# kkrt-labs/stwo-brainfuck

Hardware: AMD Instinct MI355X
Metric: trace cells committed+proved/sec (higher is better)
Workload: dtype u32 (M31 / QM31 modular arithmetic)

## Files before the change

### bindings/rust/bfhip_sys.rs

```rust
#![allow(non_camel_case_types, dead_code)]
use std::ffi::{c_char, c_void};

#[repr(C)] pub struct BfhipCtx { _private: [u8; 0] }
#[repr(C)] pub struct BfhipTrace { _private: [u8; 0] }
#[repr(C)] #[derive(Clone, Copy, Default, Debug, PartialEq, Eq)] pub struct BfhipConventions { pub merkle_node_hash: u32, pub mix_u64: u32, pub logup_mask_order: u32, pub merkle_channel: u32, pub reserved: [u32; 4] }
#[repr(C)] #[derive(Clone, Copy, Debug, PartialEq, Eq)] pub struct BfhipPcsConfig { pub pow_bits: u32, pub log_blowup_factor: u32, pub log_last_layer_degree_bound: u32, pub n_queries: u32, pub reserved: [u32; 4] }
#[repr(C)] pub struct BfhipLocalGroup { _private: [u8; 0] }
#[repr(C)] pub struct BfhipPool { _private: [u8; 0] }

#[link(name = "bfhip")]
extern "C" {
    pub fn bfhip_last_error() -> *const c_char;
    pub fn bfhip_device_count() -> i32;
    pub fn bfhip_device_memory(device_id: i32, free_bytes: *mut u64, total_bytes: *mut u64) -> i32;
    pub fn bfhip_ctx_create(device_id: i32, max_log_domain: u32, out: *mut *mut BfhipCtx) -> i32;
    pub fn bfhip_ctx_destroy(ctx: *mut BfhipCtx) -> i32;
    pub fn bfhip_ctx_sync(ctx: *mut BfhipCtx) -> i32;
    pub fn bfhip_ctx_set_overlap(ctx: *mut BfhipCtx, mask: u32) -> i32;
    pub fn bfhip_ctx_memory(ctx: *mut BfhipCtx, out: *mut u64) -> i32;
    pub fn bfhip_ctx_set_sync_policy(ctx: *mut BfhipCtx, blocking: i32) -> i32;
    pub fn bfhip_ctx_set_mailbox(ctx: *mut BfhipCtx, mode: i32, timeout_ms: u32, test_delay_ms: i32) -> i32;
    pub fn bfhip_ctx_set_conventions(ctx: *mut BfhipCtx, conv: *const BfhipConventions) -> i32;
    pub fn bfhip_ctx_get_conventions(ctx: *mut BfhipCtx, out: *mut BfhipConventions) -> i32;
    pub fn bfhip_ctx_set_pcs_config(ctx: *mut BfhipCtx, pcs: *const BfhipPcsConfig) -> i32;
// ... 2 lines not shown
    pub fn bfhip_free(ctx: *mut BfhipCtx, ptr_d: *mut c_void) -> i32;
    pub fn bfhip_upload(ctx: *mut BfhipCtx, dst_d: *mut c_void, src_h: *const c_void, bytes: usize) -> i32;
    pub fn bfhip_download(ctx: *mut BfhipCtx, dst_h: *mut c_void, src_d: *const c_void, bytes: usize) -> i32;
    pub fn bfhip_memset_zero(ctx: *mut BfhipCtx, dst_d: *mut c_void, bytes: usize) -> i32;
    pub fn bfhip_twiddles(ctx: *mut BfhipCtx, tw_d: *mut *const u32, itw_d: *mut *const u32, root_log: *mut u32) -> i32;
    pub fn bfhip_interpolate(ctx: *mut BfhipCtx, src_cols_h: *const *mut u32, dst_cols_h: *const *mut u32, n_cols: u32, log_size: u32, replicated: i32) -> i32;
    pub fn bfhip_evaluate(ctx: *mut BfhipCtx, coeff_cols_h: *const *mut u32, dst_cols_h: *const *mut u32, n_cols: u32, log_size: u32, log_eval: u32, replicated: i32) -> i32;
    pub fn bfhip_is_first_coeffs(ctx: *mut BfhipCtx, log_min: u32, log_max: u32, dst_cols_h: *const *mut u32) -> i32;
    pub fn bfhip_broadcast16(ctx: *mut BfhipCtx, rows_d: *const u32, dst_d: *mut u32, n_rows: usize) -> i32;
    pub fn bfhip_bit_reverse(ctx: *mut BfhipCtx, src_d: *const u32, dst_d: *mut u32, log_size: u32) -> i32;
    pub fn bfhip_batch_inverse_m31(ctx: *mut BfhipCtx, src_d: *const u32, dst_d: *mut u32, n: usize) -> i32;
    pub fn bfhip_batch_inverse_qm31(ctx: *mut BfhipCtx, src_d: *const *const u32, dst_d: *const *mut u32, n: usize) -> i32;
    pub fn bfhip_accumulate(ctx: *mut BfhipCtx, dst_d: *mut u32, src_d: *const u32, n: usize) -> i32;
    pub fn bfhip_eval_at_point(ctx: *mut BfhipCtx, coeffs_d: *const u32, log_size: u32, replicated: i32, point_h: *const u32, out_h: *mut u32) -> i32;
    pub fn bfhip_merkle_commit_layer(ctx: *mut BfhipCtx, log_size: u32, prev_layer_d: *const c_void, cols_h: *const *const u32, col_shifts_h: *const u32, n_cols: u32, out_hashes_d: *mut c_void) -> i32;
    pub fn bfhip_merkle_commit_layer_poseidon252(ctx: *mut BfhipCtx, log_size: u32, prev_layer_d: *const c_void, cols_h: *const *const u32, col_shifts_h: *const u32, n_cols: u32, out_hashes_d: *mut c_void) -> i32;
    pub fn bfhip_hades_permutation(ctx: *mut BfhipCtx, in_h: *const u32, out_h: *mut u32) -> i32;
    pub fn bfhip_fold_line(ctx: *mut BfhipCtx, src_d: *const *const u32, dst_d: *const *mut u32, log_size: u32, alpha_h: *const u32) -> i32;
    pub fn bfhip_fold_circle_into_line(ctx: *mut BfhipCtx, dst_d: *const *mut u32, src_d: *const *const u32, log_size: u32, alpha_h: *const u32) -> i32;
    pub fn bfhip_grind(ctx: *mut BfhipCtx, digest_h: *const u8, pow_bits: u32, nonce: *mut u64) -> i32;
    pub fn bfhip_gather(ctx: *mut BfhipCtx, col_d: *const u32, idx_h: *const u64, n: usize, out_h: *mut u32) -> i32;
    pub fn bfhip_component_shape(component: i32, n_main_cols: *mut u32, n_logup_cols: *mut u32, n_constraints: *mut u32) -> i32;
    pub fn bfhip_logup_generate(ctx: *mut BfhipCtx, component: i32, log_size: u32, main_rows_h: *const *const u32, lookup_h: *const u32, out_cols_h: *const *mut u32, claimed_sum_h: *mut u32) -> i32;
    pub fn bfhip_eval_constraints(ctx: *mut BfhipCtx, component: i32, log_size: u32, is_first_d: *const u32, main_lde_h: *const *const u32, main_shifts_h: *const u32, inter_lde_h: *const *const u32, inter_shifts_h: *const u32, lookup_h: *const u32, claimed_sum_h: *const u32, coeffs_h: *const u32, acc_d: *const *mut u32) -> i32;
    pub fn bfhip_accumulate_quotients(ctx: *mut BfhipCtx, log_size: u32, cols_h: *const *const u32, col_shifts_h: *const u32, n_cols: u32, n_samples_h: *const u32, sample_points_h: *const u32, sample_values_h: *const u32, random_coeff_h: *const u32, out_d: *const *mut u32) -> i32;
    pub fn bfhip_prove_brainfuck(ctx: *mut BfhipCtx, code: *const c_char, input_h: *const u8, n_input: usize, log_max_rows: u32, proof_json: *mut *mut c_char, proof_len: *mut usize, transcript: *mut *mut c_char, phase_seconds: *mut f64) -> i32;
    pub fn bfhip_free_host(p: *mut c_void);
    pub fn bfhip_ctx_last_proof_flags(ctx: *mut BfhipCtx, flags: *mut u32) -> i32;
    pub fn bfhip_local_group_create(count: u32, out: *mut *mut BfhipLocalGroup) -> i32;
    pub fn bfhip_local_group_destroy(group: *mut BfhipLocalGroup) -> i32;
// ... 42 lines not shown
```

### include/bfhip.h

```cpp
#ifndef BFHIP_H
#define BFHIP_H
#include <stdint.h>
#include <stddef.h>

#ifdef __cplusplus
extern "C" {
#endif

typedef struct bfhip_ctx bfhip_ctx;
typedef struct bfhip_trace bfhip_trace;

enum { BFHIP_MERKLE_STWO_COMPRESS = 0, BFHIP_MERKLE_RFC7693 = 1 };
enum { BFHIP_MIX_U64_COMPRESS = 0, BFHIP_MIX_U64_HASH = 1 };
enum { BFHIP_LOGUP_MASK_CUR_PREV = 0, BFHIP_LOGUP_MASK_PREV_CUR = 1 };
enum { BFHIP_CHANNEL_BLAKE2S = 0, BFHIP_CHANNEL_POSEIDON252 = 1 };
typedef struct bfhip_conventions {
    uint32_t merkle_node_hash;
    uint32_t mix_u64;
    uint32_t logup_mask_order;
    uint32_t merkle_channel;
    uint32_t reserved[4];
} bfhip_conventions;

const char* bfhip_last_error(void);
// ... 32 lines not shown

int32_t bfhip_interpolate(bfhip_ctx* ctx, uint32_t* const* src_cols_h, uint32_t* const* dst_cols_h, uint32_t n_cols, uint32_t log_size, int32_t replicated);
int32_t bfhip_evaluate(bfhip_ctx* ctx, uint32_t* const* coeff_cols_h, uint32_t* const* dst_cols_h, uint32_t n_cols, uint32_t log_size, uint32_t log_eval, int32_t replicated);

int32_t bfhip_is_first_coeffs(bfhip_ctx* ctx, uint32_t log_min, uint32_t log_max, uint32_t* const* dst_cols_h);


int32_t bfhip_broadcast16(bfhip_ctx* ctx, const uint32_t* rows_d, uint32_t* dst_d, size_t n_rows);
int32_t bfhip_bit_reverse(bfhip_ctx* ctx, const uint32_t* src_d, uint32_t* dst_d, uint32_t log_size);
int32_t bfhip_batch_inverse_m31(bfhip_ctx* ctx, const uint32_t* src_d, uint32_t* dst_d, size_t n);
int32_t bfhip_batch_inverse_qm31(bfhip_ctx* ctx, const uint32_t* const src_d[4], uint32_t* const dst_d[4], size_t n);
int32_t bfhip_accumulate(bfhip_ctx* ctx, uint32_t* dst_d, const uint32_t* src_d, size_t n);
int32_t bfhip_eval_at_point(bfhip_ctx* ctx, const uint32_t* coeffs_d, uint32_t log_size, int32_t replicated, const uint32_t point_h[8], uint32_t out_h[4]);
int32_t bfhip_merkle_commit_layer(bfhip_ctx* ctx, uint32_t log_size, const void* prev_layer_d, const uint32_t* const* cols_h, const uint32_t* col_shifts_h,
                                  uint32_t n_cols, void* out_hashes_d);
int32_t bfhip_merkle_commit_layer_poseidon252(bfhip_ctx* ctx, uint32_t log_size, const void* prev_layer_d, const uint32_t* const* cols_h,
                                             const uint32_t* col_shifts_h, uint32_t n_cols, void* out_hashes_d);
int32_t bfhip_hades_permutation(bfhip_ctx* ctx, const uint32_t in_h[24], uint32_t out_h[24]);
int32_t bfhip_fold_line(bfhip_ctx* ctx, const uint32_t* const src_d[4], uint32_t* const dst_d[4], uint32_t log_size, const uint32_t alpha_h[4]);
int32_t bfhip_fold_circle_into_line(bfhip_ctx* ctx, uint32_t* const dst_d[4], const uint32_t* const src_d[4], uint32_t log_size, const uint32_t alpha_h[4]);
int32_t bfhip_grind(bfhip_ctx* ctx, const uint8_t digest_h[32], uint32_t pow_bits, uint64_t* nonce);
int32_t bfhip_gather(bfhip_ctx* ctx, const uint32_t* col_d, const uint64_t* idx_h, size_t n, uint32_t* out_h);


int32_t bfhip_component_shape(int32_t component, uint32_t* n_main_cols, uint32_t* n_logup_cols, uint32_t* n_constraints);
int32_t bfhip_logup_generate(bfhip_ctx* ctx, int32_t component, uint32_t log_size, const uint32_t* const* main_rows_h, const uint32_t lookup_h[24],
                             uint32_t* const* out_cols_h, uint32_t claimed_sum_h[4]);
int32_t bfhip_eval_constraints(bfhip_ctx* ctx, int32_t component, uint32_t log_size, const uint32_t* is_first_d, const uint32_t* const* main_lde_h,
                               const uint32_t* main_shifts_h, const uint32_t* const* inter_lde_h, const uint32_t* inter_shifts_h, const uint32_t lookup_h[24],
                               const uint32_t claimed_sum_h[4], const uint32_t* coeffs_h, uint32_t* const acc_d[4]);
// ... 76 lines not shown
```

### stwo-brainfuck_amd/__init__.py

```python
import ctypes
import os
import weakref

import numpy as np

_HERE = os.path.dirname(os.path.abspath(__file__))
_LIB_PATH = os.environ.get("BFHIP_LIBRARY") or os.path.join(_HERE, "libbfhip.so")
TESTHOOKS_LIBRARY = os.path.join(_HERE, "libbfhip_testhooks.so")
_lib = None

P = (1 << 31) - 1


class BfhipError(RuntimeError):
    pass


def lib():
    global _lib
    if _lib is None:
        if not os.path.exists(_LIB_PATH):
            raise BfhipError(f"{_LIB_PATH} is missing: build it with __graft_entry__.build(); there is no CPU fallback")
        _lib = ctypes.CDLL(_LIB_PATH)
        _lib.bfhip_last_error.restype = ctypes.c_char_p
# ... 250 lines not shown
    def bit_reverse(self, src_ptr, dst_ptr, log_size):
        _check(lib().bfhip_bit_reverse(self._h, ctypes.c_void_p(src_ptr), ctypes.c_void_p(dst_ptr), log_size))

    def batch_inverse_m31(self, src_ptr, dst_ptr, n):
        _check(lib().bfhip_batch_inverse_m31(self._h, ctypes.c_void_p(src_ptr), ctypes.c_void_p(dst_ptr), ctypes.c_size_t(n)))

    def batch_inverse_qm31(self, src_ptrs, dst_ptrs, n):
        _check(lib().bfhip_batch_inverse_qm31(self._h, self._ptr_array(src_ptrs), self._ptr_array(dst_ptrs), ctypes.c_size_t(n)))

    def accumulate(self, dst_ptr, src_ptr, n):
        _check(lib().bfhip_accumulate(self._h, ctypes.c_void_p(dst_ptr), ctypes.c_void_p(src_ptr), ctypes.c_size_t(n)))

    def merkle_commit_layer(self, log_size, prev_ptr, col_ptrs, out_ptr, col_shifts=None):
        sh = None if col_shifts is None else (ctypes.c_uint32 * len(col_shifts))(*col_shifts)
        _check(lib().bfhip_merkle_commit_layer(self._h, log_size, ctypes.c_void_p(prev_ptr) if prev_ptr else None, self._ptr_array(col_ptrs), sh, len(col_ptrs), ctypes.c_void_p(out_ptr)))

    def merkle_commit_layer_poseidon252(self, log_size, prev_ptr, col_ptrs, out_ptr, col_shifts=None):
        sh = None if col_shifts is None else (ctypes.c_uint32 * len(col_shifts))(*col_shifts)
        _check(lib().bfhip_merkle_commit_layer_poseidon252(self._h, log_size, ctypes.c_void_p(prev_ptr) if prev_ptr else None, self._ptr_array(col_ptrs), sh, len(col_ptrs), ctypes.c_void_p(out_ptr)))

    def hades_permutation(self, state3):
        words = []
        for x in state3:
            words += [(int(x) >> (32 * i)) & 0xFFFFFFFF for i in range(8)]
        out = (ctypes.c_uint32 * 24)()
        _check(lib().bfhip_hades_permutation(self._h, (ctypes.c_uint32 * 24)(*words), out))
        return [sum(int(out[8 * k + i]) << (32 * i) for i in range(8)) for k in range(3)]

    def fold_line(self, src_ptrs, dst_ptrs, log_size, alpha4):
        _check(lib().bfhip_fold_line(self._h, self._ptr_array(src_ptrs), self._ptr_array(dst_ptrs), log_size, (ctypes.c_uint32 * 4)(*[int(v) for v in alpha4])))
# ... 217 lines not shown
```

### stwo-brainfuck_amd/csrc/api.hip

```cpp
#include "../../include/bfhip.h"
#include "ctx.h"
#include <cstdlib>
#include "host/circle.h"
#include "host/quotients.h"
#include <cstdio>
#include <vector>
#include <algorithm>
#include <chrono>

using namespace bf;

static thread_local std::string g_err;
void bfhip_set_error(const std::string& s) { g_err = s; }

#define API_TRY try {
#define API_CTX(ctx) try { if (!(ctx)) throw HipError("null context"); (ctx)->c.bind();
#define API_CATCH } catch (const std::exception& e) { g_err = e.what(); return -1; } catch (...) { g_err = "unknown error"; return -1; }

namespace bf {

void Ctx::ensure_aux() { for (auto& a : aux) if (!a) BF_HIP(hipStreamCreateWithFlags(&a, hipStreamNonBlocking)); }
void Ctx::ensure_side() { if (!stream2) BF_HIP(hipStreamCreateWithFlags(&stream2, hipStreamNonBlocking)); }

void Ctx::init(int dev, u32 max_log_domain, const Ctx* tables_from) {
// ... 767 lines not shown
        case 9: r = q_mul_const(x, q_const(y)); break;
        default: r = q_inv(x); break;
    }
    out[4 * i] = r.a.a; out[4 * i + 1] = r.a.b; out[4 * i + 2] = r.b.a; out[4 * i + 3] = r.b.b;
}
extern "C" int32_t bfhip_test_field_op(bfhip_ctx* ctx, uint32_t op, const uint32_t* a_d, const uint32_t* b_d, uint32_t* out_d, size_t n) {
    API_CTX(ctx)
    if (op > 10) throw HipError("bfhip_test_field_op: unknown op");
    if (!a_d || !b_d || !out_d) throw HipError("null argument");
    if (n == 0 || n > (size_t(1) << 28)) throw HipError("bfhip_test_field_op: n out of range");
    hipLaunchKernelGGL(k_test_field_op, dim3((u32)((n + 255) / 256)), dim3(256), 0, ctx->c.stream, op, a_d, b_d, out_d, (u32)n);
    BF_HIP(hipGetLastError());
    return 0;
    API_CATCH
}
extern "C" int32_t bfhip_test_constraint_group_rows(int32_t component, uint32_t log_size, uint32_t main_shift) {
    if (component < 0 || component >= N_COMPONENTS) { g_err = "unknown component"; return -1; }
    ConstraintLaunch L{};
    for (u32 j = 0; j < n_main_cols(component); j++) L.trace[j].shift = main_shift;
    for (u32 j = 0; j + 4 < 4 * n_logup_cols(component); j++) L.inter[j].shift = main_shift;
    L.log_size = log_size;
    return (int32_t)constraint_group_rows(L, component);
}
#endif
```

### stwo-brainfuck_amd/csrc/ctx.h

```cpp
#pragma once
#include <cstdlib>
#include <thread>
#include <chrono>
#include "kernels.h"
#include "comm.h"
#include <memory>
#include <vector>
#include <string>
#include <stdexcept>
#include <cstring>

namespace bf {

struct HipError : std::runtime_error { using std::runtime_error::runtime_error; };
#define BF_HIP(expr) do { hipError_t e__ = (expr); if (e__ != hipSuccess) { (void)hipGetLastError(); throw bf::HipError(std::string(#expr) + ": " + hipGetErrorString(e__)); } } while (0)

struct Arena {
    struct Chunk { char* base; size_t size, used; };
    std::vector<Chunk> chunks;
    size_t chunk_bytes = size_t(1) << 30;
    size_t total_used = 0, peak = 0;
    void* alloc(size_t bytes) {
        bytes = (bytes + 255) & ~size_t(255);
        for (auto& c : chunks) if (c.size - c.used >= bytes) { void* p = c.base + c.used; c.used += bytes; total_used += bytes; if (total_used > peak) peak = total_used; return p; }
// ... 34 lines not shown
    void ensure_aux();
    hipStream_t id_main = nullptr;
    hipStream_t aux_of(hipStream_t s) const { return s == id_main ? aux[0] : aux[1]; }
    hipEvent_t evp[32] = {};
    u32 evp_next = 0;
    hipEvent_t next_event() { return evp[evp_next++ % 32]; }
    u32* d_counters = nullptr;
    u32* merkle_counter() { return d_counters + 64 * (stream == id_main ? 0 : stream == aux[0] ? 1 : stream == aux[1] ? 2 : 3); }
    hipEvent_t ev[6] = {nullptr, nullptr, nullptr, nullptr, nullptr, nullptr};
    u32 tw_root_log = 0;
    u32* d_tw = nullptr; u32* d_itw = nullptr;
    bool owns_tables = true;
    const struct SharedPreprocessed* shared_pre = nullptr;
    uint2* d_tlo = nullptr; uint2* d_thi = nullptr;
    Arena arena;
    char* h_small = nullptr; size_t h_small_bytes = 256 << 10;
    char* d_small_alias = nullptr; char* d_hstage_alias = nullptr;
    template <class T> T* small_alias(T* host_ptr) const { return reinterpret_cast<T*>(d_small_alias + (reinterpret_cast<char*>(host_ptr) - h_small)); }
    char* h_stage = nullptr; char* d_stage = nullptr; size_t stage_bytes = 8 << 20, stage_used = 0;
    u32 last_proof_flags = 0;
    u32 proof_seq = 0;
    int mailbox_mode = -1;
    bool use_mailbox = false;
    int mailboxes_pending = 0;
    double mailbox_timeout = 10.0;
    int mailbox_test_delay_ms = 0;
    u32* flag_host(int k) const { return reinterpret_cast<u32*>(h_small + 3072 + 64 * k); }
    u32* stamp_host(int k) const { return reinterpret_cast<u32*>(h_small + 3584 + 64 * k); }
    u32* mailbox_err_host() const { return reinterpret_cast<u32*>(h_small + 3520); }
    hipEvent_t reap_ev[64] = {}; u32 reap_head = 0, reap_tail = 0;
// ... 147 lines not shown
```

### stwo-brainfuck_amd/csrc/kernels.h

```cpp
#pragma once
#include <hip/hip_runtime.h>
#include "m31.h"
#include "air.h"
#include <string>
#include <vector>

namespace bf {

struct ColDesc { const u32* ptr; u32 shift; u32 pad_; };

int prof_mode(hipStream_t s);
void prof_enable(hipStream_t s, int mode);
void prof_run_begin(hipStream_t s, const char* name);
void prof_run_end(hipStream_t s);
void prof_begin(hipStream_t s, const char* name, double bytes, double units, double aux = 0.0);
void prof_end(hipStream_t s);
void prof_reset(hipStream_t s);
std::string prof_report_json(const hipStream_t* streams, int n);
void prof_forget(hipStream_t s);
struct ProfScope {
    hipStream_t s; bool on;
    ProfScope(hipStream_t s_, const char* name, double bytes, double units = 0.0, bool dominant = false, double aux = 0.0) : s(s_) {
        int m = prof_mode(s);
        on = m == 1 || (m == 2 && dominant);
// ... 43 lines not shown
    const u32* tw;
    u32 block0, grid_x;
    u32 kind;
};
struct FftLaunch { int kind; u32 first_group, ngroups, total_blocks; double bytes, alg, bfly; };
struct FftPlan { bool inverse = false; std::vector<PassArgs> groups; std::vector<FftLaunch> launches; const PassArgs* d_groups = nullptr; };
void fft_plan(FftPlan& plan, bool inverse, const FftJob* jobs, size_t njobs, const u32* tw, const u32* itw, u32 tw_root_log);
void fft_run(hipStream_t stream, const FftPlan& plan);

struct IsFirstCols { u32* ptr[28]; u32 log_min, log_max; };
void is_first_coeffs(hipStream_t stream, const IsFirstCols& a, const u32* itw, u32 tw_root_log);

void merkle_layer(hipStream_t stream, void* out, const void* prev, const ColDesc* d_cols, u32 ncols, u32 log, double col_bytes, u32 out_shift, u32 prev_shift,
                  u32 node_conv, u32 first = 0, u32 count = 0);
struct MerkleTreeDesc { uint4* layers[32]; u32 shifts[32]; u32 col_off[32]; const ColDesc* cols; u32 n_cols, max_log; };
static constexpr u32 MERKLE_SUBTREE_ROOT_LEVEL = 9;
void merkle_subtree(hipStream_t stream, const MerkleTreeDesc& tree, u32 hi, u32 node_conv, double bytes, double compressions);
void merkle_subtree_share(hipStream_t stream, const MerkleTreeDesc& tree, u32 hi, u32 stop, u32 lo, u32 wg0, u32 n_wg, u32 node_conv, double bytes, double compressions);
void merkle_top(hipStream_t stream, const MerkleTreeDesc& tree, u32 top_hi, u32 node_conv, u32* d_chan, u32* d_alpha8, u32* d_root_copy, double bytes, double compressions,
                u32* d_stamp = nullptr, u32 stamp_value = 0);
struct FriTailLayer {
    u32* ev[4];
    const u32* quot[4];
    uint4* tree[11];
};
struct FriTailArgs {
    u32 n_layers, top_log;
    u32 alpha_idx, root_idx;
    u32* ev_last[4];
    u32* chan; u32* alpha; u32* roots;
// ... 71 lines not shown
```

### stwo-brainfuck_amd/csrc/merkle.hip

```cpp
#include "kernels.h"
#include <stdexcept>

namespace bf {

__device__ __constant__ const u32 B2S_IV[8] = {0x6A09E667u, 0xBB67AE85u, 0x3C6EF372u, 0xA54FF53Au, 0x510E527Fu, 0x9B05688Cu, 0x1F83D9ABu, 0x5BE0CD19u};

__device__ __forceinline__ u32 rotr(u32 x, int r) { return __builtin_amdgcn_alignbit(x, x, r); }

#define B2S_G(a, b, c, d, x, y) \
    a = a + b + (x); d = rotr(d ^ a, 16); c = c + d; b = rotr(b ^ c, 12); \
    a = a + b + (y); d = rotr(d ^ a, 8);  c = c + d; b = rotr(b ^ c, 7);

#define B2S_ROUND(s0, s1, s2, s3, s4, s5, s6, s7, s8, s9, s10, s11, s12, s13, s14, s15) \
    B2S_G(v0, v4, v8, v12, m[s0], m[s1]) B2S_G(v1, v5, v9, v13, m[s2], m[s3])           \
    B2S_G(v2, v6, v10, v14, m[s4], m[s5]) B2S_G(v3, v7, v11, v15, m[s6], m[s7])         \
    B2S_G(v0, v5, v10, v15, m[s8], m[s9]) B2S_G(v1, v6, v11, v12, m[s10], m[s11])       \
    B2S_G(v2, v7, v8, v13, m[s12], m[s13]) B2S_G(v3, v4, v9, v14, m[s14], m[s15])

__device__ __forceinline__ void blake2s_compress(u32 h[8], const u32 m[16], u32 t0, u32 f0) {
    u32 v0 = h[0], v1 = h[1], v2 = h[2], v3 = h[3], v4 = h[4], v5 = h[5], v6 = h[6], v7 = h[7];
    u32 v8 = 0x6A09E667u, v9 = 0xBB67AE85u, v10 = 0x3C6EF372u, v11 = 0xA54FF53Au;
    u32 v12 = 0x510E527Fu ^ t0, v13 = 0x9B05688Cu, v14 = 0x1F83D9ABu ^ f0, v15 = 0x5BE0CD19u;
    B2S_ROUND(0, 1, 2, 3, 4, 5, 6, 7, 8, 9, 10, 11, 12, 13, 14, 15)
    B2S_ROUND(14, 10, 4, 8, 9, 15, 13, 6, 1, 12, 0, 2, 11, 7, 5, 3)
// ... 249 lines not shown
                u32 ha, hb;
                node_hash_quad(ha, hb, has, ka, kb, kc, kd, cols, ncols, i, rfc, qi);
                u32* o = reinterpret_cast<u32*>(td.layers[lg]) + 8 * (size_t)i; o[qi] = ha; o[4 + qi] = hb;
                u32* l = reinterpret_cast<u32*>(s_lv[lg & 1]) + 8 * j; l[qi] = ha; l[4 + qi] = hb;
            } else {
                u32 h[8];
                node_hash_lean(h, has, ka, kb, kc, kd, cols, ncols, i, rfc);
                hash_to_hbm(td.layers[lg], i, h);
                hash_to_lds(s_lv[lg & 1], j, h);
            }
        }
        __syncthreads();
    }
}

__global__ void __launch_bounds__(256) k_merkle_top(const MerkleTreeDesc td, u32 top_hi, u32* chan, u32* alpha_out, u32* root_out, u32 rfc, u32* stamp_out, u32 stamp_value) {
    __shared__ uint4 s_lv[2][2 * 512];
    __shared__ u32 s_ch[16];
    const u32 t = threadIdx.x, qi = t & 3, qn = t >> 2;
    if (chan && t < 8) s_ch[t] = chan[t];
    u32 n_sent = 0;
    for (int lg = (int)top_hi;;) {
        const bool tree = lg >= 0;
        const ColDesc* cols = tree ? td.cols + td.col_off[lg] : nullptr;
        const u32 ncols = tree ? (lg > 0 ? td.col_off[lg - 1] : td.n_cols) - td.col_off[lg] : 0u;
        const bool first = lg == (int)top_hi, has = !first || top_hi < td.max_log;
        const uint4* prev = tree && first && has ? td.layers[lg + 1] : nullptr;
        const uint4* src = s_lv[(lg + 1) & 1];
        const u32 n = tree ? 1u << lg : 1u;
        const bool quad = !tree || n <= 64;
// ... 300 lines not shown
#ifndef MERKLE_NODES_PER_LANE
#define MERKLE_NODES_PER_LANE 4
#endif
void merkle_layer(hipStream_t stream, void* out, const void* prev, const ColDesc* d_cols, u32 ncols, u32 log, double col_bytes, u32 out_shift, u32 prev_shift,
                  u32 node_conv, u32 first, u32 count) {
    const u32 total = (1u << log) >> out_shift;
    const u32 n = count ? count : total;
    u32 threads = n < 256 ? (n < 64 ? 64 : n) : 256;
    const double frac = (double)n / (double)total;
    const double comp_per_node = (prev ? 1.0 : 0.0) + (double)((ncols + 15) / 16) + ((!prev && ncols == 0) ? 1.0 : 0.0);
    ProfScope ps(stream, "k_merkle_layer", ((prev ? 64.0 * total : 0.0) + 32.0 * total + col_bytes) * frac, comp_per_node * n, true);
    u32 blocks = (n + threads - 1) / threads;
    if (blocks >= (1u << 14)) blocks /= MERKLE_NODES_PER_LANE;
    hipLaunchKernelGGL(k_merkle_layer, dim3(blocks), dim3(threads), 0, stream, (uint4*)out, (const uint4*)prev, d_cols, ncols, n, out_shift, prev_shift, count ? first : 0u, node_conv ? 0xFFFFFFFFu : 0u);
}
void merkle_subtree(hipStream_t stream, const MerkleTreeDesc& tree, u32 hi, u32 node_conv, double bytes, double compressions) {
    ProfScope ps(stream, "k_merkle_subtree", bytes, compressions);
    hipLaunchKernelGGL(k_merkle_subtree, dim3(1u << MERKLE_SUBTREE_ROOT_LEVEL), dim3(256), 0, stream, tree, hi, node_conv ? 0xFFFFFFFFu : 0u,
                       (u32)MERKLE_SUBTREE_ROOT_LEVEL, (u32)MERKLE_SUBTREE_ROOT_LEVEL, 0u);
}
void merkle_subtree_share(hipStream_t stream, const MerkleTreeDesc& tree, u32 hi, u32 stop, u32 lo, u32 wg0, u32 n_wg, u32 node_conv, double bytes, double compressions) {
    if (hi < stop || stop < lo || hi - lo > 9 || !n_wg) throw std::runtime_error("merkle_subtree_share: bad level range");
    ProfScope ps(stream, "k_merkle_subtree", bytes, compressions);
    hipLaunchKernelGGL(k_merkle_subtree, dim3(n_wg), dim3(256), 0, stream, tree, hi, node_conv ? 0xFFFFFFFFu : 0u, lo, stop, wg0);
}
void merkle_top(hipStream_t stream, const MerkleTreeDesc& tree, u32 top_hi, u32 node_conv, u32* d_chan, u32* d_alpha8, u32* d_root_copy, double bytes, double compressions,
                u32* d_stamp, u32 stamp_value) {
    ProfScope ps(stream, "k_merkle_top", bytes, compressions);
    hipLaunchKernelGGL(k_merkle_top, dim3(1), dim3(256), 0, stream, tree, top_hi, d_chan, d_alpha8, d_root_copy, node_conv ? 0xFFFFFFFFu : 0u, d_stamp, stamp_value);
}
// ... 74 lines not shown
```

### stwo-brainfuck_amd/csrc/prover.hip

```cpp
#include <atomic>
#include "../../include/bfhip.h"
#include "ctx.h"
#include "host/circle.h"
#include "host/quotients.h"
#include "host/proof.h"
#include "host/verifier.h"
#include <map>
#include <set>
#include <chrono>
#include <algorithm>
#include <cstdio>
#include <functional>
#include <mutex>

namespace bf {

void build_tables_device(Ctx& c, const std::vector<u32> trace7_soa[7], u32 n, const std::vector<u32>& code, const std::function<u32*(size_t)>& alloc,
                         std::vector<std::vector<u32*>>& cols_out, u32 log_sizes_out[13]);

static constexpr u32 OWNER_ALL = 0xFFFFFFFFu;

struct DCol {
    u32* ptr = nullptr; u32 log_size = 0; u32 shift = 0;
    u32 lc = 0;
// ... 162 lines not shown
    }

    template <class F> void stage_blocks(Mailbox* mbx, F&& f) {
        if (mbx) { mbx->begin(); f(); mbx->arm(); }
        else { StageBatch sb(c); f(); sb.end(); }
    }

    struct ChannelStep { u32* chan; u32* alpha8; u32* root_copy; };
    struct MerklePlan {
        DevMerkle mk; std::vector<DCol> cols; std::vector<size_t> off; std::vector<double> bytes; size_t n_all = 0;
        const ColDesc* d_all = nullptr; MerkleTreeDesc tree{}; bool poseidon = false;
        u32 fused_top = 0, sub_hi = 0;
        double top_bytes = 0, top_comp = 0, sub_bytes = 0, sub_comp = 0;
        int band_fuse_hi = -1; u32 band_fuse_r = 0; double band_bytes = 0, band_comp = 0;
    };
    MerklePlan merkle_plan(const std::vector<DCol>& cols_in) {
        if (cols_in.empty()) throw HipError("merkle_commit: no columns");
        MerklePlan p;
        p.cols = cols_in;
        std::vector<DCol>& cols = p.cols;
        std::stable_sort(cols.begin(), cols.end(), [](const DCol& a, const DCol& b) { return a.log_size > b.log_size; });
        DevMerkle& mk = p.mk;
        mk.cols = cols;
        mk.max_log = cols[0].log_size;
        mk.layers.resize(mk.max_log + 1);
        mk.shifts.assign(mk.max_log + 1, 0);
        u32 min_col_log = cols.back().log_size;
        std::vector<ColDesc> all; p.off.assign(mk.max_log + 2, 0); p.bytes.assign(mk.max_log + 1, 0.0);
        {
            size_t ci = 0;
            for (int log = (int)mk.max_log; log >= 0; log--) {
// ... 10 lines not shown
        while (fused_top > 0 && mk.shifts[std::min(fused_top, mk.max_log)] != 0) fused_top--;
        if (p.poseidon) fused_top = 0;
        p.fused_top = fused_top;
        const ShardGroup& sg = c.shard;
        if (sg.count > 1) {
            const int share_min = p.poseidon ? 8 : (int)SHARE_MIN_LOG_PER_RANK;
            int lo = std::max<int>((int)sg.log_count + share_min, (int)fused_top);
            while (lo <= (int)mk.max_log && (int)lo - (int)mk.shifts[lo] < (int)sg.log_count + share_min) lo++;
            const bool worth = (int)mk.max_log - (int)mk.shifts[mk.max_log] >= (int)sg.log_count + (int)SLICE_MIN_LOG_PER_RANK;
            if (worth && lo <= (int)mk.max_log) { mk.band_hi = (int)mk.max_log; mk.band_lo = lo; }
            for (auto& col : cols) if (col.sliced() && ((int)col.log_size < mk.band_lo || (int)col.log_size > mk.band_hi)) throw HipError("shard group: a row-sharded column lies outside the share-wise Merkle band");
        }
        const bool banded = mk.band_hi >= mk.band_lo;
        for (int log = (int)mk.max_log; log >= 0; log--) {
            const size_t stored = (size_t(1) << log) >> mk.shifts[log];
            if (banded && log > mk.band_lo && log <= mk.band_hi) {
                const size_t per_rank = stored >> sg.log_count;
                mk.layers[log] = reinterpret_cast<u32*>(reinterpret_cast<uintptr_t>(c.arena.alloc(32 * per_rank)) - 32 * per_rank * sg.rank);
            } else mk.layers[log] = (u32*)c.arena.alloc(32 * stored);
        }
        if (fused_top == 10 && mk.max_log >= 11) {
            u32 hi = std::min<u32>(banded ? (u32)mk.band_lo - 1 : mk.max_log, 17);
            while (hi > 10 && mk.shifts[hi] != 0) hi--;
            if (hi > 10) { p.sub_hi = hi; p.fused_top = fused_top = MERKLE_SUBTREE_ROOT_LEVEL; }
        }
        auto level_cols = [&](int log) { return (log > 0 ? p.off[log - 1] : all.size()) - p.off[log]; };
        auto level_cost = [&](int log, double& bytes, double& comp) {
            const double nodes = (double)(1u << log), nc = (double)level_cols(log);
            const bool has = log < (int)mk.max_log;
            bytes += nodes * ((has ? 64.0 : 0.0) + 32.0) + p.bytes[log];
            comp += nodes * ((has ? 1.0 : 0.0) + (double)(((u32)nc + 15) / 16) + ((!has && nc == 0) ? 1.0 : 0.0));
        };
        if (banded && !p.poseidon && fused_top > 0 && mk.band_hi > mk.band_lo && c.shard.band_fusion) {
            const int hi = std::min(mk.band_hi, mk.band_lo + 3);
            bool plain = true;
            for (int lg = mk.band_lo; lg <= std::min(hi + 1, (int)mk.max_log); lg++) plain = plain && mk.shifts[lg] == 0;
            const u32 r = 8 - (u32)(hi - mk.band_lo);
            if (plain && (u32)mk.band_lo >= sg.log_count + r) {
                p.band_fuse_hi = hi; p.band_fuse_r = r;
                for (int lg = hi; lg >= mk.band_lo; lg--) level_cost(lg, p.band_bytes, p.band_comp);
                p.band_bytes /= sg.count; p.band_comp /= sg.count;
            }
        }
        for (int log = (int)fused_top - 1; log >= 0; log--) level_cost(log, p.top_bytes, p.top_comp);
        if (p.sub_hi) for (int log = (int)p.sub_hi; log >= (int)MERKLE_SUBTREE_ROOT_LEVEL; log--) level_cost(log, p.sub_bytes, p.sub_comp);
        p.d_all = all.empty() ? nullptr : c.stage(all.data(), all.size());
        if (fused_top > 0) {
// ... 4 lines not shown
            p.tree = td;
        }
        return p;
    }
    struct LevelWait { int level; hipEvent_t ev; };
    DevMerkle merkle_run(MerklePlan& p, Hash32* pinned_root = nullptr, bool no_readback = false, const ChannelStep* step = nullptr, const std::vector<LevelWait>* waits = nullptr,
                         int stamp_slot = -1, bool* stamped = nullptr) {
        DevMerkle& mk = p.mk;
        const ShardGroup& sg = c.shard;
        const bool poseidon = p.poseidon;
        const u32 fused_top = p.fused_top;
        if (poseidon && step) throw HipError("the device-side channel step is a Blake2s path");
        const char* layer_kernel = poseidon ? "k_merkle_layer_poseidon" : "k_merkle_layer";
        prof_run_begin(c.stream, layer_kernel);
        const int single_lo = p.sub_hi ? (int)p.sub_hi + 1 : (int)fused_top;
        size_t wi = 0;
        auto apply_waits = [&](int log) { while (waits && wi < waits->size() && (*waits)[wi].level >= log) BF_HIP(hipStreamWaitEvent(c.stream, (*waits)[wi++].ev, 0)); };
        for (int log = (int)mk.max_log; log >= single_lo; log--) {
            apply_waits(log);
            if (log == p.band_fuse_hi) {
                prof_run_end(c.stream);
                const u32 n_wg = ((1u << mk.band_lo) >> sg.log_count) >> p.band_fuse_r;
                merkle_subtree_share(c.stream, p.tree, (u32)log, (u32)mk.band_lo, (u32)mk.band_lo - p.band_fuse_r, sg.rank * n_wg, n_wg, c.conv.merkle_node_hash, p.band_bytes, p.band_comp);
                sg.comm->all_gather(c.stream, mk.layers[mk.band_lo], (size_t(32) << mk.band_lo) >> sg.log_count);
                prof_run_begin(c.stream, layer_kernel);
                log = mk.band_lo;
                continue;
            }
            size_t n = (log > 0 ? p.off[log - 1] : p.n_all) - p.off[log];
            const bool share = log >= mk.band_lo && log <= mk.band_hi;
            const u32 per_rank = share ? ((1u << (log - mk.shifts[log])) >> sg.log_count) : 0u;
            if (poseidon)
                merkle_layer_poseidon(c.stream, mk.layers[log], log < (int)mk.max_log ? mk.layers[log + 1] : nullptr, n ? p.d_all + p.off[log] : nullptr, (u32)n, (u32)log,
                                      mk.shifts[log], log < (int)mk.max_log ? mk.shifts[log + 1] : 0, sg.rank * per_rank, per_rank);
            else
                merkle_layer(c.stream, mk.layers[log], log < (int)mk.max_log ? mk.layers[log + 1] : nullptr, n ? p.d_all + p.off[log] : nullptr, (u32)n, (u32)log, p.bytes[log],
                             mk.shifts[log], log < (int)mk.max_log ? mk.shifts[log + 1] : 0, c.conv.merkle_node_hash, sg.rank * per_rank, per_rank);
            if (share && log == mk.band_lo) {
                prof_run_end(c.stream);
                sg.comm->all_gather(c.stream, mk.layers[log], ((size_t(32) << log) >> mk.shifts[log]) >> sg.log_count);
                prof_run_begin(c.stream, layer_kernel);
// ... 1342 lines not shown
    try {
        if (!ctx || !t || !n_rows) { bfhip_set_error("null argument"); return -1; }
        if (component >= N_COMPONENTS || column >= t->in.rows[component].size()) { bfhip_set_error("bad component/column"); return -1; }
        const DCol& col = t->in.rows[component][column];
        *n_rows = col.stored();
        if (out_h) {
            if (cap < col.stored()) { bfhip_set_error("capacity"); return -2; }
            ctx->c.bind();
            BF_HIP(hipMemcpyAsync(out_h, col.ptr, col.stored() * sizeof(u32), hipMemcpyDeviceToHost, ctx->c.stream));
            ctx->c.sync();
        }
        return 0;
    } catch (const std::exception& e) { bfhip_set_error(e.what()); return -1; }
}

static void release_group_after_failure(bfhip_ctx* ctx) {
    if (ctx && ctx->c.shard.count > 1 && ctx->c.shard.comm) {
        try { ctx->c.shard.comm->abort(); } catch (...) {}
        Ctx& c = ctx->c;
        for (hipStream_t st : {c.stream, c.id_main, c.stream2, c.aux[0], c.aux[1]}) if (st) (void)hipStreamSynchronize(st);
    }
}

static void fill_outputs(HipProver& pv, const BrainfuckProof& bp, char** proof_json, size_t* proof_len, char** transcript, double* phase_seconds) {
    if (proof_json) {
        std::string js = proof_to_json(bp, pv.c.conv.merkle_channel == 1);
        *proof_json = (char*)malloc(js.size() + 1);
        memcpy(*proof_json, js.c_str(), js.size() + 1);
        if (proof_len) *proof_len = js.size();
    }
// ... 199 lines not shown
```

Baseline: 14.27 billion.

## Fuse up to four Blake2s Merkle levels into one LDS-staged kernel

Adds k_merkle_levels, which hashes two to four consecutive unreplicated Merkle levels (up to level 21) in one launch. Child hashes pass between levels through shared memory instead of global round trips, and the prover groups eligible levels above the subtree using a new planner that respects bands and wait events. The aim is to cut per-level launch overhead and global memory traffic for the mid-sized layers. The cost is lower parallelism per level inside a block, and idle waves at the deeper fused levels. Also adds a merkle_commit_tree API and a test knob for the fusion ceiling.

After: 14.11 billion. 0.989x the previous value.

```diff
diff --git a/bindings/rust/bfhip_sys.rs b/bindings/rust/bfhip_sys.rs
--- a/bindings/rust/bfhip_sys.rs
+++ b/bindings/rust/bfhip_sys.rs
@@ -40,6 +40,7 @@
     pub fn bfhip_accumulate(ctx: *mut BfhipCtx, dst_d: *mut u32, src_d: *const u32, n: usize) -> i32;
     pub fn bfhip_eval_at_point(ctx: *mut BfhipCtx, coeffs_d: *const u32, log_size: u32, replicated: i32, point_h: *const u32, out_h: *mut u32) -> i32;
     pub fn bfhip_merkle_commit_layer(ctx: *mut BfhipCtx, log_size: u32, prev_layer_d: *const c_void, cols_h: *const *const u32, col_shifts_h: *const u32, n_cols: u32, out_hashes_d: *mut c_void) -> i32;
+    pub fn bfhip_merkle_commit_tree(ctx: *mut BfhipCtx, cols_h: *const *const u32, log_sizes_h: *const u32, col_shifts_h: *const u32, n_cols: u32, layers_h: *const *mut c_void, level_shifts_h: *mut u32, root_h: *mut u8) -> i32;
     pub fn bfhip_merkle_commit_layer_poseidon252(ctx: *mut BfhipCtx, log_size: u32, prev_layer_d: *const c_void, cols_h: *const *const u32, col_shifts_h: *const u32, n_cols: u32, out_hashes_d: *mut c_void) -> i32;
     pub fn bfhip_hades_permutation(ctx: *mut BfhipCtx, in_h: *const u32, out_h: *mut u32) -> i32;
     pub fn bfhip_fold_line(ctx: *mut BfhipCtx, src_d: *const *const u32, dst_d: *const *mut u32, log_size: u32, alpha_h: *const u32) -> i32;
diff --git a/include/bfhip.h b/include/bfhip.h
--- a/include/bfhip.h
+++ b/include/bfhip.h
@@ -70,6 +70,8 @@
 int32_t bfhip_eval_at_point(bfhip_ctx* ctx, const uint32_t* coeffs_d, uint32_t log_size, int32_t replicated, const uint32_t point_h[8], uint32_t out_h[4]);
 int32_t bfhip_merkle_commit_layer(bfhip_ctx* ctx, uint32_t log_size, const void* prev_layer_d, const uint32_t* const* cols_h, const uint32_t* col_shifts_h,
                                   uint32_t n_cols, void* out_hashes_d);
+int32_t bfhip_merkle_commit_tree(bfhip_ctx* ctx, const uint32_t* const* cols_h, const uint32_t* log_sizes_h, const uint32_t* col_shifts_h, uint32_t n_cols,
+                                 void* const* layers_h, uint32_t* level_shifts_h, uint8_t root_h[32]);
 int32_t bfhip_merkle_commit_layer_poseidon252(bfhip_ctx* ctx, uint32_t log_size, const void* prev_layer_d, const uint32_t* const* cols_h,
                                              const uint32_t* col_shifts_h, uint32_t n_cols, void* out_hashes_d);
 int32_t bfhip_hades_permutation(bfhip_ctx* ctx, const uint32_t in_h[24], uint32_t out_h[24]);
diff --git a/stwo-brainfuck_amd/__init__.py b/stwo-brainfuck_amd/__init__.py
--- a/stwo-brainfuck_amd/__init__.py
+++ b/stwo-brainfuck_amd/__init__.py
@@ -288,6 +288,17 @@
     def merkle_commit_layer(self, log_size, prev_ptr, col_ptrs, out_ptr, col_shifts=None):
         sh = None if col_shifts is None else (ctypes.c_uint32 * len(col_shifts))(*col_shifts)
         _check(lib().bfhip_merkle_commit_layer(self._h, log_size, ctypes.c_void_p(prev_ptr) if prev_ptr else None, self._ptr_array(col_ptrs), sh, len(col_ptrs), ctypes.c_void_p(out_ptr)))
+
+    def merkle_commit_tree(self, col_ptrs, log_sizes, layer_ptrs, col_shifts=None):
+        n, nl = len(col_ptrs), max(log_sizes) + 1
+        if len(layer_ptrs) < nl:
+            raise BfhipError("merkle_commit_tree: one layer pointer per level 0 .. max(log_sizes)")
+        logs = (ctypes.c_uint32 * n)(*log_sizes)
+        sh = (ctypes.c_uint32 * n)(*col_shifts) if col_shifts else None
+        layers = (ctypes.c_void_p * nl)(*layer_ptrs[:nl])
+        shifts, root = (ctypes.c_uint32 * nl)(), (ctypes.c_uint8 * 32)()
+        _check(lib().bfhip_merkle_commit_tree(self._h, self._ptr_array(col_ptrs), logs, sh, n, layers, shifts, root))
+        return bytes(root), list(shifts)
 
     def merkle_commit_layer_poseidon252(self, log_size, prev_ptr, col_ptrs, out_ptr, col_shifts=None):
         sh = None if col_shifts is None else (ctypes.c_uint32 * len(col_shifts))(*col_shifts)
diff --git a/stwo-brainfuck_amd/csrc/api.hip b/stwo-brainfuck_amd/csrc/api.hip
--- a/stwo-brainfuck_amd/csrc/api.hip
+++ b/stwo-brainfuck_amd/csrc/api.hip
@@ -805,6 +805,11 @@
     return 0;
     API_CATCH
 }
+extern "C" int32_t bfhip_test_set_merkle_fuse_max_hi(bfhip_ctx* ctx, uint32_t level) {
+    if (!ctx) { g_err = "null context"; return -1; }
+    ctx->c.merkle_fuse_max_hi = level;
+    return 0;
+}
 extern "C" int32_t bfhip_test_constraint_group_rows(int32_t component, uint32_t log_size, uint32_t main_shift) {
     if (component < 0 || component >= N_COMPONENTS) { g_err = "unknown component"; return -1; }
     ConstraintLaunch L{};
diff --git a/stwo-brainfuck_amd/csrc/ctx.h b/stwo-brainfuck_amd/csrc/ctx.h
--- a/stwo-brainfuck_amd/csrc/ctx.h
+++ b/stwo-brainfuck_amd/csrc/ctx.h
@@ -72,6 +72,7 @@
     const struct SharedPreprocessed* shared_pre = nullptr;
     uint2* d_tlo = nullptr; uint2* d_thi = nullptr;
     Arena arena;
+    u32 merkle_fuse_max_hi = MERKLE_FUSE_MAX_HI;
     char* h_small = nullptr; size_t h_small_bytes = 256 << 10;
     char* d_small_alias = nullptr; char* d_hstage_alias = nullptr;
     template <class T> T* small_alias(T* host_ptr) const { return reinterpret_cast<T*>(d_small_alias + (reinterpret_cast<char*>(host_ptr) - h_small)); }
diff --git a/stwo-brainfuck_amd/csrc/host/merkle_groups.h b/stwo-brainfuck_amd/csrc/host/merkle_groups.h
--- /dev/null
+++ b/stwo-brainfuck_amd/csrc/host/merkle_groups.h
@@ -0,0 +1,25 @@
+#pragma once
+#include <cstdint>
+#include <vector>
+
+namespace bf {
+
+struct MerkleLevelGroup { int hi; int n; };
+
+static constexpr int MERKLE_GROUP_MAX_LEVELS = 4;
+
+inline std::vector<MerkleLevelGroup> merkle_level_groups(int lo, int hi, const uint32_t* shifts, int band_lo, int band_hi, const std::vector<int>& wait_levels, int fuse_max_hi) {
+    auto fusable = [&](int lg) { return lg <= fuse_max_hi && shifts[lg] == 0 && !(band_hi >= band_lo && lg >= band_lo && lg <= band_hi); };
+    auto waits_at = [&](int lg) { for (int w : wait_levels) if (w == lg) return true; return false; };
+    std::vector<MerkleLevelGroup> up;
+    for (int lg = lo; lg <= hi;) {
+        int n = 1;
+        if (fusable(lg))
+            while (n < MERKLE_GROUP_MAX_LEVELS && lg + n <= hi && fusable(lg + n) && !waits_at(lg + n - 1)) n++;
+        up.push_back({lg + n - 1, n});
+        lg += n;
+    }
+    return std::vector<MerkleLevelGroup>(up.rbegin(), up.rend());
+}
+
+}
diff --git a/stwo-brainfuck_amd/csrc/kernels.h b/stwo-brainfuck_amd/csrc/kernels.h
--- a/stwo-brainfuck_amd/csrc/kernels.h
+++ b/stwo-brainfuck_amd/csrc/kernels.h
@@ -81,6 +81,8 @@
 void merkle_layer(hipStream_t stream, void* out, const void* prev, const ColDesc* d_cols, u32 ncols, u32 log, double col_bytes, u32 out_shift, u32 prev_shift,
                   u32 node_conv, u32 first = 0, u32 count = 0);
 struct MerkleTreeDesc { uint4* layers[32]; u32 shifts[32]; u32 col_off[32]; const ColDesc* cols; u32 n_cols, max_log; };
+static constexpr u32 MERKLE_FUSE_MAX_HI = 21;
+void merkle_levels(hipStream_t stream, const MerkleTreeDesc& tree, u32 hi, u32 nlev, u32 node_conv, double bytes, double compressions);
 static constexpr u32 MERKLE_SUBTREE_ROOT_LEVEL = 9;
 void merkle_subtree(hipStream_t stream, const MerkleTreeDesc& tree, u32 hi, u32 node_conv, double bytes, double compressions);
 void merkle_subtree_share(hipStream_t stream, const MerkleTreeDesc& tree, u32 hi, u32 stop, u32 lo, u32 wg0, u32 n_wg, u32 node_conv, double bytes, double compressions);
diff --git a/stwo-brainfuck_amd/csrc/merkle.hip b/stwo-brainfuck_amd/csrc/merkle.hip
--- a/stwo-brainfuck_amd/csrc/merkle.hip
+++ b/stwo-brainfuck_amd/csrc/merkle.hip
@@ -287,6 +287,74 @@
     }
 }
 
+__device__ __forceinline__ void levels_first_block(u32 (&m)[16], const uint4* __restrict__ prev, u32 ps, const ColDesc* __restrict__ cols, u32 ncols, u32 i) {
+    if (prev) {
+        const size_t cl = ((size_t)2 * i) >> ps, cr = ((size_t)2 * i + 1) >> ps;
+        kids_to_m(m, prev[2 * cl], prev[2 * cl + 1], prev[2 * cr], prev[2 * cr + 1]);
+    } else if (ncols) load_col_words<4>(m, cols, 0, ncols, i);
+    else {
+#pragma unroll
+        for (u32 w = 0; w < 16; w++) m[w] = 0;
+    }
+}
+__global__ void __launch_bounds__(256) k_merkle_levels(const MerkleTreeDesc td, u32 hi, u32 nlev, u32 rfc) {
+    __shared__ u32 s_lv[8 * 768];
+    const u32 t = threadIdx.x, wave = (u32)__builtin_amdgcn_readfirstlane((int)(t >> 6)), lane = t & 63, rot = blockIdx.x & 3;
+    const bool top_has = hi < td.max_log;
+    const uint4* prev = top_has ? td.layers[hi + 1] : nullptr;
+    const u32 ps = top_has ? td.shifts[hi + 1] : 0u;
+    u32 nx[16];
+#pragma unroll 1
+    for (u32 lv = 0; lv < nlev; lv++) {
+        const u32 lg = hi - lv, n = 512u >> lv;
+        const ColDesc* cols = td.cols + td.col_off[lg];
+        const u32 ncols = td.col_off[lg - 1] - td.col_off[lg];
+        const bool has = lv > 0 || top_has, pre = has || ncols <= 4;
+        const u32 total_bytes = (has ? 64u : 0u) + 4u * ncols;
+        const u32 vw = (wave - (lv == 2 ? rot : lv == 3 ? rot + 2 : 0u)) & 3;
+        u32* dst = (lv & 1) ? s_lv + 512 : s_lv;
+        const u32* src = (lv & 1) ? s_lv : s_lv + 512;
+#pragma unroll 1
+        for (int it = lv == 0 ? -1 : 0; it < (lv == 0 ? 2 : 1); it++) {
+            const u32 j0 = vw * 64 + 256 * (u32)it, j = j0 + lane;
+            if (it < 0 || j0 < n) {
+                const u32 i = (blockIdx.x << (9 - lv)) + j;
+                u32 m[16], h[8];
+                if (lv == 0) {
+#pragma unroll
+                    for (u32 w = 0; w < 16; w++) m[w] = it < 0 ? 0u : nx[w];
+                    if (it < 1 && pre) levels_first_block(nx, prev, ps, cols, ncols, i + 256);
+                    if (it < 0) continue;
+                } else {
+#pragma unroll
+                    for (u32 w = 0; w < 8; w++) { const uint2 p = *reinterpret_cast<const uint2*>(src + w * 768 + 2 * j); m[w] = p.x; m[8 + w] = p.y; }
+                }
+                node_init(h, rfc);
+                u32 done = 0, c0 = 0;
+                bool last = false;
+                if (pre) {
+                    done = has ? 64u : total_bytes;
+                    last = done == total_bytes;
+                    blake2s_compress(h, m, done & rfc, last ? rfc : 0u);
+                }
+#pragma unroll 1
+                while (!last) {
+                    load_col_block(m, cols, c0, ncols, i);
+                    c0 += 16; done += min(64u, total_bytes - done);
+                    last = done == total_bytes;
+                    blake2s_compress(h, m, done & rfc, last ? rfc : 0u);
+                }
+                store_hash(td.layers[lg], i, h);
+                if (lv + 1 < nlev) {
+#pragma unroll
+                    for (u32 w = 0; w < 8; w++) dst[w * 768 + j] = h[w];
+                }
+            }
+        }
+        if (lv + 1 < nlev) __syncthreads();
+    }
+}
+
 __global__ void __launch_bounds__(256) k_merkle_top(const MerkleTreeDesc td, u32 top_hi, u32* chan, u32* alpha_out, u32* root_out, u32 rfc, u32* stamp_out, u32 stamp_value) {
     __shared__ uint4 s_lv[2][2 * 512];
     __shared__ u32 s_ch[16];
@@ -617,6 +685,12 @@
     if (blocks >= (1u << 14)) blocks /= MERKLE_NODES_PER_LANE;
     hipLaunchKernelGGL(k_merkle_layer, dim3(blocks), dim3(threads), 0, stream, (uint4*)out, (const uint4*)prev, d_cols, ncols, n, out_shift, prev_shift, count ? first : 0u, node_conv ? 0xFFFFFFFFu : 0u);
 }
+void merkle_levels(hipStream_t stream, const MerkleTreeDesc& tree, u32 hi, u32 nlev, u32 node_conv, double bytes, double compressions) {
+    if (nlev < 2 || nlev > 4 || hi > tree.max_log || hi < 9 + nlev) throw std::runtime_error("merkle_levels: bad level range");
+    for (u32 lg = hi - nlev + 1; lg <= hi; lg++) if (tree.shifts[lg]) throw std::runtime_error("merkle_levels: replicated level");
+    ProfScope ps(stream, "k_merkle_layer", bytes, compressions, true);
+    hipLaunchKernelGGL(k_merkle_levels, dim3(1u << (hi - 9)), dim3(256), 0, stream, tree, hi, nlev, node_conv ? 0xFFFFFFFFu : 0u);
+}
 void merkle_subtree(hipStream_t stream, const MerkleTreeDesc& tree, u32 hi, u32 node_conv, double bytes, double compressions) {
     ProfScope ps(stream, "k_merkle_subtree", bytes, compressions);
     hipLaunchKernelGGL(k_merkle_subtree, dim3(1u << MERKLE_SUBTREE_ROOT_LEVEL), dim3(256), 0, stream, tree, hi, node_conv ? 0xFFFFFFFFu : 0u,
diff --git a/stwo-brainfuck_amd/csrc/prover.hip b/stwo-brainfuck_amd/csrc/prover.hip
--- a/stwo-brainfuck_amd/csrc/prover.hip
+++ b/stwo-brainfuck_amd/csrc/prover.hip
@@ -5,6 +5,7 @@
 #include "host/quotients.h"
 #include "host/proof.h"
 #include "host/verifier.h"
+#include "host/merkle_groups.h"
 #include <map>
 #include <set>
 #include <chrono>
@@ -200,7 +201,13 @@
         double top_bytes = 0, top_comp = 0, sub_bytes = 0, sub_comp = 0;
         int band_fuse_hi = -1; u32 band_fuse_r = 0; double band_bytes = 0, band_comp = 0;
     };
-    MerklePlan merkle_plan(const std::vector<DCol>& cols_in) {
+    static void merkle_level_cost(const MerklePlan& p, int log, double& bytes, double& comp) {
+        const double nodes = (double)(1u << log), nc = (double)((log > 0 ? p.off[log - 1] : p.n_all) - p.off[log]);
+        const bool has = log < (int)p.mk.max_log;
+        bytes += nodes * ((has ? 64.0 : 0.0) + 32.0) + p.bytes[log];
+        comp += nodes * ((has ? 1.0 : 0.0) + (double)(((u32)nc + 15) / 16) + ((!has && nc == 0) ? 1.0 : 0.0));
+    }
+    MerklePlan merkle_plan(const std::vector<DCol>& cols_in, void* const* layers_out = nullptr) {
         if (cols_in.empty()) throw HipError("merkle_commit: no columns");
         MerklePlan p;
         p.cols = cols_in;
@@ -241,6 +248,7 @@
         const bool banded = mk.band_hi >= mk.band_lo;
         for (int log = (int)mk.max_log; log >= 0; log--) {
             const size_t stored = (size_t(1) << log) >> mk.shifts[log];
+            if (layers_out) { mk.layers[log] = (u32*)layers_out[log]; continue; }
             if (banded && log > mk.band_lo && log <= mk.band_hi) {
                 const size_t per_rank = stored >> sg.log_count;
                 mk.layers[log] = reinterpret_cast<u32*>(reinterpret_cast<uintptr_t>(c.arena.alloc(32 * per_rank)) - 32 * per_rank * sg.rank);
@@ -251,13 +259,7 @@
             while (hi > 10 && mk.shifts[hi] != 0) hi--;
             if (hi > 10) { p.sub_hi = hi; p.fused_top = fused_top = MERKLE_SUBTREE_ROOT_LEVEL; }
         }
-        auto level_cols = [&](int log) { return (log > 0 ? p.off[log - 1] : all.size()) - p.off[log]; };
-        auto level_cost = [&](int log, double& bytes, double& comp) {
-            const double nodes = (double)(1u << log), nc = (double)level_cols(log);
-            const bool has = log < (int)mk.max_log;
-            bytes += nodes * ((has ? 64.0 : 0.0) + 32.0) + p.bytes[log];
-            comp += nodes * ((has ? 1.0 : 0.0) + (double)(((u32)nc + 15) / 16) + ((!has && nc == 0) ? 1.0 : 0.0));
-        };
+        auto level_cost = [&](int log, double& bytes, double& comp) { merkle_level_cost(p, log, bytes, comp); };
         if (banded && !p.poseidon && fused_top > 0 && mk.band_hi > mk.band_lo && c.shard.band_fusion) {
             const int hi = std::min(mk.band_hi, mk.band_lo + 3);
             bool plain = true;
@@ -292,6 +294,12 @@
         const char* layer_kernel = poseidon ? "k_merkle_layer_poseidon" : "k_merkle_layer";
         prof_run_begin(c.stream, layer_kernel);
         const int single_lo = p.sub_hi ? (int)p.sub_hi + 1 : (int)fused_top;
+        unsigned char grp_n[33] = {};
+        if (!poseidon && p.sub_hi) {
+            std::vector<int> wait_levels;
+            if (waits) for (auto& w : *waits) wait_levels.push_back(w.level);
+            for (auto& g : merkle_level_groups(single_lo, (int)mk.max_log, mk.shifts.data(), mk.band_lo, mk.band_hi, wait_levels, (int)c.merkle_fuse_max_hi)) grp_n[g.hi] = (unsigned char)g.n;
+        }
         size_t wi = 0;
         auto apply_waits = [&](int log) { while (waits && wi < waits->size() && (*waits)[wi].level >= log) BF_HIP(hipStreamWaitEvent(c.stream, (*waits)[wi++].ev, 0)); };
         for (int log = (int)mk.max_log; log >= single_lo; log--) {
@@ -303,6 +311,13 @@
                 sg.comm->all_gather(c.stream, mk.layers[mk.band_lo], (size_t(32) << mk.band_lo) >> sg.log_count);
                 prof_run_begin(c.stream, layer_kernel);
                 log = mk.band_lo;
+                continue;
+            }
+            if (grp_n[log] >= 2) {
+                double bytes = 0, comp = 0;
+                for (int lg = log; lg > log - (int)grp_n[log]; lg--) merkle_level_cost(p, lg, bytes, comp);
+                merkle_levels(c.stream, p.tree, (u32)log, grp_n[log], c.conv.merkle_node_hash, bytes, comp);
+                log -= (int)grp_n[log] - 1;
                 continue;
             }
             size_t n = (log > 0 ? p.off[log - 1] : p.n_all) - p.off[log];
@@ -1675,6 +1690,35 @@
     } catch (const std::exception& e) { bfhip_set_error(e.what()); return -1; }
 }
 
+extern "C" int32_t bfhip_merkle_commit_tree(bfhip_ctx* ctx, const uint32_t* const* cols_h, const uint32_t* log_sizes_h, const uint32_t* col_shifts_h, uint32_t n_cols,
+                                             void* const* layers_h, uint32_t* level_shifts_h, uint8_t root_h[32]) {
+    try {
+        if (!ctx) throw HipError("null context");
+        if (!cols_h || !log_sizes_h || !layers_h || !n_cols) throw HipError("null argument");
+        Ctx& c = ctx->c;
+        c.bind();
+        if (c.shard.count > 1) throw HipError("bfhip_merkle_commit_tree: not for a context of a shard group");
+        std::vector<DCol> cols(n_cols);
+        u32 max_log = 0;
+        for (u32 k = 0; k < n_cols; k++) {
+            const u32 sh = col_shifts_h ? col_shifts_h[k] : 0u;
+            if (!cols_h[k] || log_sizes_h[k] > 30 || sh > log_sizes_h[k]) throw HipError("bfhip_merkle_commit_tree: bad column");
+            cols[k].ptr = const_cast<u32*>(cols_h[k]); cols[k].log_size = log_sizes_h[k]; cols[k].shift = sh;
+            max_log = std::max(max_log, log_sizes_h[k]);
+        }
+        for (u32 lg = 0; lg <= max_log; lg++) if (!layers_h[lg]) throw HipError("bfhip_merkle_commit_tree: null level");
+        HipProver pv(c, 0);
+        c.stage_checkpoint();
+        StageBatch sb(c);
+        HipProver::MerklePlan p = pv.merkle_plan(cols, layers_h);
+        sb.end();
+        DevMerkle mk = pv.merkle_run(p);
+        if (level_shifts_h) for (u32 lg = 0; lg <= max_log; lg++) level_shifts_h[lg] = mk.shifts[lg];
+        if (root_h) memcpy(root_h, mk.root.b, 32);
+        return 0;
+    } catch (const std::exception& e) { bfhip_set_error(e.what()); return -1; } catch (...) { bfhip_set_error("unknown error"); return -1; }
+}
+
 static void release_group_after_failure(bfhip_ctx* ctx) {
     if (ctx && ctx->c.shard.count > 1 && ctx->c.shard.comm) {
         try { ctx->c.shard.comm->abort(); } catch (...) {}
```
